# ctb/khmer

Measured on NVIDIA B200. Metric: kmers_per_sec_countgraph_k20_N4, higher is better.
Workload: dtype u8

## Files before the change

khmer_b200/csrc/kmgpu_api.cu:

```cuda
#include <algorithm>
#include <cstdarg>
#include <cstdio>
#include <cstdlib>
#include <cstring>
#include <chrono>
#include <functional>
#include <mutex>
#include <string>
#include <unordered_map>
#include <vector>

#include "../../include/kmgpu.h"
#include "kmgpu_kernels.cuh"
#include "kmgpu_group.cuh"

using namespace kmgpu;

static thread_local std::string g_err;

static int fail(int code, const char* fmt, ...)
{
    char buf[1024];
    va_list ap;
    va_start(ap, fmt);
// ... 942 lines not shown
        for (const Part& pt : parts) {
            const Input& in = pt.in;
            if (in.n_pos == 0) continue;
            const unsigned gt = n_tiles(in.n_pos);
            if (src == 1) k_bigscan2<TWOBIT, 1><<<gt, THREADS, 0, st>>>(h->dev, H, in, sg, h->d_htkeys.p, slots - 1, n_cross ? 1 : 0, h->d_events.p,
                                                                       (unsigned long long)cap, h->d_ctrl, pt.pos_off, MM, PP, pred ? 1 : 0);
            else if (H.kind == TWOBIT) k_bigscan2<TWOBIT, 0><<<gt, THREADS, 0, st>>>(h->dev, H, in, sg, h->d_htkeys.p, slots - 1, n_cross ? 1 : 0, h->d_events.p,
                                                                                   (unsigned long long)cap, h->d_ctrl, pt.pos_off, MM, PP, pred ? 1 : 0);
            else k_bigscan2<MURMUR, 0><<<gt, THREADS, 0, st>>>(h->dev, H, in, sg, h->d_htkeys.p, slots - 1, n_cross ? 1 : 0, h->d_events.p,
                                                             (unsigned long long)cap, h->d_ctrl, pt.pos_off, MM, PP, pred ? 1 : 0);
            h->all_launches += 1;
        }
    }
    SatBits sb;
    memset(&sb, 0, sizeof sb);
    for (int i = 0; i < h->nt && i < F_MAXT; i++) sb.t[i] = h->d_satbits[i].p;
    for (size_t pi = 0; pi < parts.size(); pi++) {
        const Part& pt = parts[pi];
        Input in = pt.in;
        if (in.n_pos == 0 || rehash) continue;
        if (pi + 1 < parts.size()) in.n_pos = std::min<uint32_t>(in.n_pos, parts[pi + 1].pos_off - pt.pos_off);
        const uint32_t* bins = h->d_bins.p + pt.pos_off;
        unsigned gb = (in.n_pos + 255) / 256;
        if (src == 1) k_bigscan<TWOBIT, 1><<<gb, 256, 0, st>>>(h->nt, H, in, bins, stride, sb, h->d_htkeys.p, slots - 1, n_cross ? 1 : 0,
                                                                h->d_events.p, (unsigned long long)cap, h->d_ctrl, pt.pos_off);
        else if (H.kind == TWOBIT) k_bigscan<TWOBIT, 0><<<gb, 256, 0, st>>>(h->nt, H, in, bins, stride, sb, h->d_htkeys.p, slots - 1,
                                                                            n_cross ? 1 : 0, h->d_events.p, (unsigned long long)cap, h->d_ctrl, pt.pos_off);
        else k_bigscan<MURMUR, 0><<<gb, 256, 0, st>>>(h->nt, H, in, bins, stride, sb, h->d_htkeys.p, slots - 1, n_cross ? 1 : 0,
                                                      h->d_events.p, (unsigned long long)cap, h->d_ctrl, pt.pos_off);
        h->all_launches += 1;
    }
    CK(cudaGetLastError());
    CKR(read_ctrl(h));
    const uint64_t n_rec = h->h_ctrl->n_events;
    lap("scan done (n_rec)", n_rec);
    if (n_rec > cap) return fail(KMGPU_ECUDA, "internal: bigcount scan overflow");
    if (n_rec == 0) return KMGPU_OK;
    const unsigned gr = (unsigned)((n_rec + 255) / 256);
    uint32_t* Tarr = nullptr;
    if (n_cross) {
        CKR(h->d_sel.ensure(std::max<uint64_t>(3 * slots, WS_MIN)));
        CKR(h->d_recslot.ensure(std::max<uint64_t>(n_rec * h->nt, 4 * WS_MIN)));
        SelState ss{h->d_sel.p, h->d_sel.p + slots, h->d_sel.p + 2 * slots};
        const unsigned gsl = (unsigned)((slots + 255) / 256);
        k_sel_slots<<<gr, 256, 0, st>>>(h->d_events.p, n_rec, h->dev, h->d_htkeys.p, slots - 1, h->d_recslot.p);
        k_sel_init<<<gsl, 256, 0, st>>>(h->d_htkeys.p, h->d_htvals.p, slots, ss);
        int top = 0;
        while (top < 31 && (1ull << (top + 1)) <= (uint64_t)n_pos) top++;
        for (int bit = top; bit >= 0; bit--) {
            k_sel_count<<<gr, 256, 0, st>>>(h->d_events.p, n_rec, h->nt, h->d_recslot.p, bit, ss);
            k_sel_update<<<gsl, 256, 0, st>>>(slots, bit, ss);
        }
        h->all_launches += 2 + 2 * (top + 1);
        Tarr = ss.prefix;
    }
    uint64_t evslots = pow2_at_least(2 * n_rec);
    CKR(h->d_evkeys.ensure(std::max<uint64_t>(evslots, WS_MIN)));
    CKR(h->d_evvals.ensure(std::max<uint64_t>(2 * evslots, 2 * WS_MIN)));
    CK(cudaMemsetAsync(h->d_evkeys.p, 0xFF, evslots * 8, st));
    CK(cudaMemsetAsync(h->d_evvals.p, 0, evslots * 4, st));
    CK(cudaMemsetAsync(h->d_evvals.p + evslots, 0xFF, evslots * 4, st));
    CK(cudaMemsetAsync(&h->d_ctrl->n_unique, 0, sizeof(unsigned long long), st));
    CK(cudaMemsetAsync(&h->d_ctrl->n_events, 0, sizeof(unsigned long long), st));
    EvTable ev{h->d_evkeys.p, h->d_evvals.p, h->d_evvals.p + evslots, evslots - 1};
    k_ev_decide<<<gr, 256, 0, st>>>(h->d_events.p, n_rec, h->nt, h->d_recslot.p, Tarr, n_cross ? 1 : 0, ev, h->d_ctrl);
    h->all_launches += 1;
    CK(cudaGetLastError());
    CKR(read_ctrl(h));
    const uint64_t n_distinct = h->h_ctrl->n_unique;
    lap("decided (n_distinct)", n_distinct);
    if (n_distinct == 0) return KMGPU_OK;
    CKR(h->d_evout.ensure(std::max<uint64_t>(n_distinct, WS_MIN / 4)));
    CKR(h->h_evout.ensure(std::max<uint64_t>(n_distinct, WS_MIN / 4)));
    k_ev_compact<<<(unsigned)((evslots + 255) / 256), 256, 0, st>>>(ev, h->d_evout.p, h->d_ctrl);
    h->all_launches += 1;
    CK(cudaGetLastError());
    CK(cudaMemcpyAsync(h->h_evout.p, h->d_evout.p, n_distinct * sizeof(EvOut), cudaMemcpyDeviceToHost, st));
    CK(cudaStreamSynchronize(st));
    std::vector<EvOut> evs(h->h_evout.p, h->h_evout.p + n_distinct);
    std::sort(evs.begin(), evs.end(), [](const EvOut& a, const EvOut& b) { return a.first < b.first; });
    for (const EvOut& e : evs) big_events(h, e.hash, e.count);
    return KMGPU_OK;
}

static bool plan_buckets(const kmgpu_sketch* h, uint32_t n_pos, BucketLayout* L)
{
    if (!env_u64("KMGPU_BUCKETS", 1)) return false;
    memset(L, 0, sizeof *L);
    L->n_tables = h->nt;
    uint64_t cap = 0, total = 0;
    for (int i = 0; i < h->nt; i++) {
        if (h->sizes[i] > 0xFFFFFFFEull - 128) return false;
        uint64_t nb = (h->sizes[i] + BKT_BINS - 1) / BKT_BINS;
        if (nb > (uint64_t)BKT_MAX_BUCKETS) return false;
        L->first[i] = (uint32_t)total;
        total += nb;
        uint64_t expect = nb == 1 ? n_pos : (uint64_t)((double)n_pos * BKT_BINS / (double)h->sizes[i]) + 1;
        cap = std::max(cap, expect + expect / 4 + 2048);
    }
    L->first[h->nt] = (uint32_t)total;
    cap = std::min<uint64_t>(cap, (uint64_t)n_pos);
    if (uint64_t forced = env_u64("KMGPU_BUCKET_CAP", 0)) cap = forced;
    if (cap > 65535 || cap == 0) return false;
    L->cap = (uint32_t)cap;
    return true;
}

template <int KIND>
static void launch_apply(unsigned g, cudaStream_t st, const SketchDev& S, const BucketLayout& L, const unsigned long long* rec, const uint32_t* cur,
                         uint32_t* newbits, uint64_t* binlist, unsigned long long list_cap, Ctrl* ctrl, int want_cross, const SatBits& sb)
{
    k_apply<KIND><<<g, 1024, BKT_APPLY_SMEM, st>>>(S, L, rec, cur, newbits, binlist, list_cap, ctrl, want_cross, sb);
}

typedef std::function<int()> Between;

#include "kmgpu_group_host.inc"

static int ingest_chunk_delta(kmgpu_sketch* h, const std::vector<DeltaPass>& passes, int src, HashCfg H, const std::vector<Part>& parts, const Pred& P,
                              bool pred, const SketchDev* M, ChunkResult* res, const Between& between)
{
    cudaStream_t st = h->stream;
    uint32_t n_pos = 0;
    for (const Part& pt : parts) n_pos = std::max(n_pos, pt.pos_off + pt.in.n_pos);
    const uint64_t stride = ((uint64_t)n_pos + 7) & ~7ull;
    CKR(h->d_bins.ensure((size_t)h->nt * stride));
    uint64_t total_bins = 0, max_span = 0;
    for (int i = 0; i < h->nt; i++) total_bins += h->sizes[i];
    for (const DeltaPass& p : passes) max_span = std::max<uint64_t>(max_span, p.hi - p.lo);
    const uint64_t list_cap = std::max<uint64_t>(1, std::min<uint64_t>((uint64_t)h->nt * n_pos, total_bins));
    CKR(h->d_binlist.ensure(list_cap));
    size_t need_lanes = h->kind == BIT ? ((max_span + 127) / 128) * 8 + 8 : ((max_span + 7) & ~7ull) + 8;
    if (h->d_delta.cap < need_lanes) h->delta_zeroed = 0;
    CKR(h->d_delta.ensure(need_lanes));
    if (h->delta_zeroed < h->d_delta.cap) {
        CK(cudaMemsetAsync(h->d_delta.p, 0, h->d_delta.cap * 2, st));
        h->delta_zeroed = h->d_delta.cap;
    }
    CK(cudaMemsetAsync(h->d_ctrl, 0, sizeof(Ctrl), st));
    CK(cudaEventRecord(h->ev0, st));
    const int want_cross = h->kind == BYTE && h->use_bigcount;
    if (want_cross && !h->satbits_valid) {
        for (int i = 0; i < h->nt; i++) {
            uint64_t groups = (h->sizes[i] + 7) / 8;
            CKR(h->d_satbits[i].ensure(groups));
            k_build_satbits<<<(unsigned)std::min<uint64_t>((groups + 255) / 256, 148 * 16), 256, 0, st>>>(h->dev.tables[i], groups, h->d_satbits[i].p);
            h->all_launches += 1;
        }
        h->satbits_valid = true;
    }
    bool kmers_counted = false;
    BucketLayout BL;
    bool use_buckets = plan_buckets(h, n_pos, &BL);
    if (use_buckets) {
        if (!h->bucket_attr_set) {
            CK(cudaFuncSetAttribute(k_bucketize<BKT_TILE, BKT_PER>, cudaFuncAttributeMaxDynamicSharedMemorySize, (int)bkt_sort_smem(BKT_TILE)));
            CK(cudaFuncSetAttribute(k_apply<BYTE>, cudaFuncAttributeMaxDynamicSharedMemorySize, (int)BKT_APPLY_SMEM));
            CK(cudaFuncSetAttribute(k_apply<NIBBLE>, cudaFuncAttributeMaxDynamicSharedMemorySize, (int)BKT_APPLY_SMEM));
            CK(cudaFuncSetAttribute(k_apply<BIT>, cudaFuncAttributeMaxDynamicSharedMemorySize, (int)BKT_APPLY_SMEM));
            h->bucket_attr_set = true;
        }
        const uint32_t n_buckets = BL.first[h->nt];
        if (h->d_records.ensure((size_t)n_buckets * BL.cap) != KMGPU_OK) {
            cudaGetLastError();
            use_buckets = false;
        }
    }
    if (use_buckets) {
        const uint32_t n_buckets = BL.first[h->nt];
        CKR(h->d_cursors.ensure(n_buckets));
        const size_t nb_words = (n_pos + 31) / 32;
        CKR(h->d_newbits.ensure(nb_words));
        CK(cudaMemsetAsync(h->d_cursors.p, 0, (size_t)n_buckets * 4, st));
        CK(cudaMemsetAsync(h->d_newbits.p, 0, nb_words * 4, st));
    }
    for (const Part& pt : parts) {
        const Input& in = pt.in;
        if (pt.ready) CK(cudaStreamWaitEvent(st, pt.ready, 0));
        if (in.n_pos == 0) continue;
        uint32_t* bins = h->d_bins.p + pt.pos_off;
        const unsigned g = n_tiles(in.n_pos);
        const SketchDev& MS = M ? *M : h->dev;
        if (src == 1) launch_hashbins<TWOBIT, 1>(pred, g, st, h->dev, MS, H, P, in, bins, stride, h->d_ctrl);
        else if (H.kind == TWOBIT) launch_hashbins<TWOBIT, 0>(pred, g, st, h->dev, MS, H, P, in, bins, stride, h->d_ctrl);
        else launch_hashbins<MURMUR, 0>(pred, g, st, h->dev, MS, H, P, in, bins, stride, h->d_ctrl);
        if (use_buckets)
            k_bucketize<BKT_TILE, BKT_PER><<<dim3((in.n_pos + BKT_TILE - 1) / BKT_TILE, h->nt), BKT_TILE / BKT_PER, bkt_sort_smem(BKT_TILE), st>>>(
                bins, stride, in.n_pos, pt.pos_off, BL, h->d_records.p, h->d_cursors.p, h->d_ctrl);
        h->ingest_launches += use_buckets ? 2 : 1;
        h->all_launches += use_buckets ? 2 : 1;
    }
    if (use_buckets) {
        const uint32_t n_buckets = BL.first[h->nt];
        const size_t nb_words = (n_pos + 31) / 32;
        SatBits sb;
        memset(&sb, 0, sizeof sb);
        if (want_cross)
            for (int i = 0; i < h->nt; i++) sb.t[i] = h->d_satbits[i].p;
        if (h->kind == BYTE) launch_apply<BYTE>(n_buckets, st, h->dev, BL, h->d_records.p, h->d_cursors.p, h->d_newbits.p, h->d_binlist.p, list_cap, h->d_ctrl, want_cross, sb);
        else if (h->kind == NIBBLE) launch_apply<NIBBLE>(n_buckets, st, h->dev, BL, h->d_records.p, h->d_cursors.p, h->d_newbits.p, h->d_binlist.p, list_cap, h->d_ctrl, 0, sb);
        else launch_apply<BIT>(n_buckets, st, h->dev, BL, h->d_records.p, h->d_cursors.p, h->d_newbits.p, h->d_binlist.p, list_cap, h->d_ctrl, 0, sb);
        k_popc<<<(unsigned)std::min<size_t>((nb_words + 255) / 256, 148 * 8), 256, 0, st>>>(h->d_newbits.p, nb_words, &h->d_ctrl->n_unique);
        CK(cudaEventRecord(h->ev1, st));
        CK(cudaGetLastError());
        if (between) CKR(between());
        CKR(read_ctrl(h));
        float ms = 0;
        CK(cudaEventElapsedTime(&ms, h->ev0, h->ev1));
        h->ingest_ms += ms;
        h->ingest_launches += 2;
        h->all_launches += 2;
        Ctrl c = *h->h_ctrl;
        res->n_kmers += c.n_kmers;
        kmers_counted = true;
        if (!c.overflow) {
            if (c.n_events > list_cap) return fail(KMGPU_ECUDA, "internal: bin list overflow");
            h->n_occupied += c.n_z0;
            if (c.n_zbits) {
                h->n_unique += c.n_unique;
                res->n_new += c.n_unique;
                res->have_newbits = true;
            }
            if (want_cross && c.n_sat) CKR(resolve_bigcount_delta(h, src, H, parts, n_pos, stride, c.n_events, c.n_cross));
            return KMGPU_OK;
        }
        if (env_u64("KMGPU_DEBUG", 0)) fprintf(stderr, "[kmgpu] bucket overflow (cap %u, %u positions): chunk redone by the delta passes\n", BL.cap, n_pos);
        CK(cudaMemsetAsync(h->d_ctrl, 0, sizeof(Ctrl), st));
        CK(cudaEventRecord(h->ev0, st));
    }
    const Between none;
    const Between& between2 = kmers_counted ? none : between;
    const unsigned gs = (n_pos + 2047) / 2048;
    for (const DeltaPass& p : passes) {
        const int pass_id = passes.size() <= 64 ? (int)(&p - passes.data()) : -1;
        if (h->kind == BIT) {
            k_scatter<true><<<gs, 256, 0, st>>>(h->d_bins.p + (size_t)p.table * stride, n_pos, p.lo, p.hi, h->d_delta.p);
            unsigned gb = (unsigned)(((uint64_t)(p.hi - p.lo) + 128 * 256 - 1) / (128 * 256));
            k_fold_bits<<<gb, 256, 0, st>>>(h->dev.tables[p.table], p.table, p.lo, p.hi, h->d_delta.p, h->d_binlist.p, list_cap, h->d_ctrl, pass_id);
            continue;
        }
        k_scatter<false><<<gs, 256, 0, st>>>(h->d_bins.p + (size_t)p.table * stride, n_pos, p.lo, p.hi, h->d_delta.p);
        unsigned gf = (unsigned)(((uint64_t)(p.hi - p.lo) + 2047) / 2048);
        if (h->kind == BYTE)
            k_fold<BYTE><<<gf, 256, 0, st>>>(h->dev.tables[p.table], p.table, p.lo, p.hi, h->d_delta.p, h->d_binlist.p, list_cap, h->d_ctrl, want_cross,
                                             want_cross ? h->d_satbits[p.table].p : nullptr, pass_id);
        else
            k_fold<NIBBLE><<<gf, 256, 0, st>>>(h->dev.tables[p.table], p.table, p.lo, p.hi, h->d_delta.p, h->d_binlist.p, list_cap, h->d_ctrl, 0, nullptr, pass_id);
    }
    CK(cudaEventRecord(h->ev1, st));
    CK(cudaGetLastError());
    if (between2) CKR(between2());
    CKR(read_ctrl(h));
    float ms = 0;
    CK(cudaEventElapsedTime(&ms, h->ev0, h->ev1));
    h->ingest_ms += ms;
    h->ingest_launches += 2 * passes.size();
    h->all_launches += 2 * passes.size();
    Ctrl c = *h->h_ctrl;
    if (c.n_events > list_cap) return fail(KMGPU_ECUDA, "internal: bin list overflow");
    if (!kmers_counted) res->n_kmers += c.n_kmers;
    h->n_occupied += c.n_z0;
    const uint64_t n_list = c.n_events;
    if (c.n_zbits) {
        size_t nb_words = (n_pos + 31) / 32;
        CKR(h->d_newbits.ensure(nb_words));
        CK(cudaMemsetAsync(h->d_newbits.p, 0, nb_words * 4, st));
        CK(cudaMemsetAsync(&h->d_ctrl->n_unique, 0, sizeof(unsigned long long), st));
        const uint64_t cold_min = env_u64("KMGPU_COLD_MIN_NEW", 8ull << 20);
        if (passes.size() <= 64 && c.n_zbits >= cold_min) {
            unsigned long long* sl = reinterpret_cast<unsigned long long*>(h->d_htkeys.p);
            uint64_t seg0 = 0;
            for (size_t pi = 0; pi < passes.size(); pi++) {
                uint64_t seg1 = seg0 + c.pass_list_end[pi];
                if (seg1 > seg0) {
                    const DeltaPass& p = passes[pi];
                    const uint32_t span = p.hi - p.lo;
                    if (span <= (1u << 26) && env_u64("KMGPU_COLD_RANK", 1)) {
                        const uint32_t n_words = (span + 31) / 32;
                        const unsigned gw = (n_words + 1023) / 1024;
                        const uint64_t n_ent = seg1 - seg0;
                        CKR(h->d_rank.ensure((size_t)n_words * 2 + gw));
                        CKR(h->d_htkeys.ensure((n_ent + 1) / 2));
                        uint2* rec = reinterpret_cast<uint2*>(h->d_rank.p);
                        uint32_t* sums = h->d_rank.p + (size_t)n_words * 2;
                        uint32_t* minpos = reinterpret_cast<uint32_t*>(h->d_htkeys.p);
                        CK(cudaMemsetAsync(rec, 0, (size_t)n_words * 8, st));
                        CK(cudaMemsetAsync(minpos, 0xFF, n_ent * 4, st));
                        unsigned gl = (unsigned)std::min<uint64_t>((n_ent + 255) / 256, 148 * 8);
                        k_rank_setbits<<<gl, 256, 0, st>>>(h->d_binlist.p + seg0, n_ent, p.lo, rec);
                        k_rank_sums<<<gw, 256, 0, st>>>(rec, n_words, sums);
                        k_rank_scan<<<1, 1024, 0, st>>>(sums, gw);
                        k_rank_prefix<<<gw, 256, 0, st>>>(rec, n_words, sums);
                        k_rank_replay<<<(n_pos + 2047) / 2048, 256, 0, st>>>(h->d_bins.p + (size_t)p.table * stride, n_pos, p.lo, p.hi, rec, minpos);
                        k_rank_mark<<<gl, 256, 0, st>>>(minpos, n_ent, h->d_newbits.p, h->d_ctrl);
                        h->all_launches += 6;
                        seg0 = seg1;
                        continue;
                    }
                    uint64_t slots = pow2_at_least(2 * (seg1 - seg0));
                    CKR(h->d_htkeys.ensure(slots));
                    sl = reinterpret_cast<unsigned long long*>(h->d_htkeys.p);
                    CK(cudaMemsetAsync(sl, 0xFF, slots * 8, st));
                    unsigned gl = (unsigned)std::min<uint64_t>((seg1 - seg0 + 255) / 256, 148 * 8);
                    k_pk_register<<<gl, 256, 0, st>>>(h->d_binlist.p + seg0, seg1 - seg0, p.table, sl, slots - 1, nullptr);
                    k_pk_replay<<<(n_pos + 1023) / 1024, 256, 0, st>>>(h->d_bins.p + (size_t)p.table * stride, n_pos, p.lo, p.hi, sl,
                                                                    slots - 1, nullptr);
                    unsigned gm = (unsigned)std::min<uint64_t>((slots + 255) / 256, 148 * 8);
                    k_pk_mark<<<gm, 256, 0, st>>>(sl, slots, h->d_newbits.p, h->d_ctrl);
                    h->all_launches += 3;
                }
                seg0 = seg1;
            }
        } else {
        PkLayout L;
        memset(&L, 0, sizeof L);
        uint64_t total_slots = 0;
        for (int i = 0; i < h->nt; i++) {
            if (!c.n_new_t[i]) continue;
            uint64_t sl = pow2_at_least(2 * c.n_new_t[i]);
            L.base[i] = total_slots;
            L.mask[i] = sl - 1;
            total_slots += sl;
        }
        L.use_filter = c.n_zbits < (uint64_t)h->nt * FILTER_BITS / 4;
        {
            uint64_t mx = 0;
            for (int i = 0; i < h->nt; i++) mx = std::max<uint64_t>(mx, c.n_new_t[i]);
            uint64_t fb = 1u << 15;
            while (fb < 32 * mx && fb < FILTER_BITS) fb <<= 1;
            L.filter_bits = (uint32_t)fb;
        }
        CKR(h->d_htkeys.ensure(total_slots));
        CK(cudaMemsetAsync(h->d_htkeys.p, 0xFF, total_slots * 8, st));
        if (L.use_filter) {
            CKR(h->d_filter.ensure((size_t)h->nt * FILTER_WORDS));
            CK(cudaMemsetAsync(h->d_filter.p, 0, (size_t)h->nt * (L.filter_bits >> 5) * 4, st));
        }
        unsigned long long* sl = reinterpret_cast<unsigned long long*>(h->d_htkeys.p);
        unsigned gl = (unsigned)std::min<uint64_t>((n_list + 255) / 256, 148 * 8);
        k_pk_register_all<<<gl, 256, 0, st>>>(h->d_binlist.p, n_list, L, sl, h->d_filter.p);
// ... 2128 lines not shown
```

khmer_b200/csrc/kmgpu_kernels.cuh:

```cuda
#pragma once
#include "kmgpu_device.cuh"

namespace kmgpu {

struct Ctrl {
    unsigned long long n_kmers;
    unsigned long long n_z0;
    unsigned long long n_zbits;
    unsigned long long n_allsat;
    unsigned long long n_sat;
    unsigned long long n_cross;
    unsigned long long n_unique;
    unsigned long long n_events;
    unsigned long long non_acgt;
    unsigned long long n_new_t[32];
    unsigned long long pass_list_end[64];
    unsigned long long overflow;
    unsigned long long queue_overflow;
};

constexpr uint32_t F_CONSUMED = 1u << 31;
constexpr int F_MAXT = 10;
constexpr uint64_t FILTER_BITS = 1ull << 23;
constexpr uint64_t FILTER_WORDS = FILTER_BITS / 32;
// ... 1062 lines not shown
    __shared__ unsigned s_w[32];
    __shared__ unsigned s_carry;
    if (threadIdx.x == 0) s_carry = 0;
    __syncthreads();
    for (uint32_t base = 0; base < n; base += 1024) {
        uint32_t i = base + threadIdx.x;
        unsigned v = i < n ? sums[i] : 0, incl = v;
        const unsigned lane = threadIdx.x & 31, wid = threadIdx.x >> 5;
#pragma unroll
        for (int o = 1; o < 32; o <<= 1) {
            unsigned t = __shfl_up_sync(0xffffffffu, incl, o);
            if (lane >= (unsigned)o) incl += t;
        }
        if (lane == 31) s_w[wid] = incl;
        __syncthreads();
        unsigned before = s_carry;
        for (unsigned w = 0; w < wid; w++) before += s_w[w];
        if (i < n) sums[i] = before + incl - v;
        __syncthreads();
        if (threadIdx.x == 1023) s_carry = before + incl;
        __syncthreads();
    }
}

__global__ void __launch_bounds__(256) k_rank_prefix(uint2* rec, uint32_t n_words, const uint32_t* __restrict__ sums)
{
    const uint32_t w0 = (blockIdx.x * 256u + threadIdx.x) * 4u;
    unsigned c[4], tot = 0;
#pragma unroll
    for (int j = 0; j < 4; j++) {
        c[j] = w0 + j < n_words ? __popc(rec[w0 + j].x) : 0;
        tot += c[j];
    }
    unsigned incl = tot;
    const unsigned lane = threadIdx.x & 31, wid = threadIdx.x >> 5;
#pragma unroll
    for (int o = 1; o < 32; o <<= 1) {
        unsigned t = __shfl_up_sync(0xffffffffu, incl, o);
        if (lane >= (unsigned)o) incl += t;
    }
    __shared__ unsigned s[8];
    if (lane == 31) s[wid] = incl;
    __syncthreads();
    unsigned at = sums[blockIdx.x] + incl - tot;
    for (unsigned w = 0; w < wid; w++) at += s[w];
#pragma unroll
    for (int j = 0; j < 4; j++) {
        if (w0 + j < n_words) rec[w0 + j].y = at;
        at += c[j];
    }
}

__global__ void __launch_bounds__(256)
k_rank_replay(const uint32_t* __restrict__ bins, uint32_t n_pos, uint32_t lo, uint32_t hi, const uint2* __restrict__ rec, uint32_t* minpos)
{
    const uint32_t p0 = (blockIdx.x * 256u + threadIdx.x) * 8u;
    if (p0 >= n_pos) return;
    uint32_t v[8];
    if (p0 + 8 <= n_pos) {
        uint4 a = __ldcs(reinterpret_cast<const uint4*>(bins + p0));
        uint4 b = __ldcs(reinterpret_cast<const uint4*>(bins + p0 + 4));
        v[0] = a.x; v[1] = a.y; v[2] = a.z; v[3] = a.w; v[4] = b.x; v[5] = b.y; v[6] = b.z; v[7] = b.w;
    } else {
#pragma unroll
        for (int j = 0; j < 8; j++) v[j] = p0 + j < n_pos ? __ldcs(bins + p0 + j) : BIN_NONE;
    }
    const uint32_t span = hi - lo;
    uint2 r[8];
#pragma unroll
    for (int j = 0; j < 8; j++) {
        v[j] -= lo;
        r[j] = v[j] < span ? __ldcg(&rec[v[j] >> 5]) : make_uint2(0, 0);
    }
#pragma unroll
    for (int j = 0; j < 8; j++) {
        const uint32_t bit = 1u << (v[j] & 31);
        if (r[j].x & bit) atomicMin(&minpos[r[j].y + __popc(r[j].x & (bit - 1))], p0 + j);
    }
}

__global__ void k_rank_mark(const uint32_t* __restrict__ minpos, uint64_t n, uint32_t* newbits, Ctrl* ctrl)
{
    unsigned cnt = 0;
    for (uint64_t i = blockIdx.x * (uint64_t)blockDim.x + threadIdx.x; i < n; i += (uint64_t)gridDim.x * blockDim.x) {
        uint32_t p = minpos[i];
        if (p == 0xFFFFFFFFu) continue;
        uint32_t bit = 1u << (p & 31);
        uint32_t old = atomicOr(&newbits[p >> 5], bit);
        cnt += !(old & bit);
    }
    cnt = __reduce_add_sync(0xffffffffu, cnt);
    if ((threadIdx.x & 31) == 0 && cnt) atomicAdd(&ctrl->n_unique, (unsigned long long)cnt);
}

struct PkLayout {
    uint64_t base[F_MAXT];
    uint64_t mask[F_MAXT];
    int use_filter;
    uint32_t filter_bits;
};

__global__ void k_pk_register_all(const uint64_t* __restrict__ binlist, uint64_t n, PkLayout L, unsigned long long* slots, uint32_t* filter)
{
    for (uint64_t i = blockIdx.x * (uint64_t)blockDim.x + threadIdx.x; i < n; i += (uint64_t)gridDim.x * blockDim.x) {
        uint64_t e = binlist[i];
        if (!(e & BL_NEW)) continue;
        int t = (int)(e & 255u);
        uint32_t bin = (uint32_t)((e & 0xFFFFFFFFFFFFull) >> 8);
        unsigned long long fresh = ((unsigned long long)bin << 32) | 0xFFFFFFFFull;
        unsigned long long* tb = slots + L.base[t];
        uint64_t s = pk_slot0(bin, L.mask[t]);
        while (true) {
            unsigned long long prev = atomicCAS(&tb[s], PK_EMPTY, fresh);
            if (prev == PK_EMPTY || (uint32_t)(prev >> 32) == bin) break;
            s = (s + 1) & L.mask[t];
        }
        if (L.use_filter) atomicOr(&filter[t * (L.filter_bits >> 5) + ((bin & (L.filter_bits - 1)) >> 5)], 1u << (bin & 31));
    }
}

__global__ void __launch_bounds__(256)
k_pk_replay_all(const uint32_t* __restrict__ bins, uint64_t stride, int n_tables, uint32_t n_pos, PkLayout L, unsigned long long* slots,
                const uint32_t* __restrict__ filter)
{
    uint32_t p = blockIdx.x * 256u + threadIdx.x;
    if (p >= n_pos) return;
    uint32_t b[F_MAXT];
    bool act[F_MAXT];
#pragma unroll
    for (int t = 0; t < F_MAXT; t++) b[t] = t < n_tables ? __ldcs(&bins[t * stride + p]) : BIN_NONE;
    if (b[0] == BIN_NONE) return;
    const uint32_t fmask = L.filter_bits - 1, fwords = L.filter_bits >> 5;
#pragma unroll
    for (int t = 0; t < F_MAXT; t++) {
        act[t] = t < n_tables && L.mask[t] != 0;
        if (act[t] && L.use_filter) act[t] = (__ldg(&filter[t * fwords + ((b[t] & fmask) >> 5)]) >> (b[t] & 31)) & 1u;
    }
#pragma unroll
    for (int t = 0; t < F_MAXT; t++) {
        if (!act[t]) continue;
        unsigned long long* tb = slots + L.base[t];
        uint64_t s = pk_slot0(b[t], L.mask[t]);
        pk_finish(tb, L.mask[t], s, __ldcg(&tb[s]), b[t], p);
    }
}

struct SatBits {
    const uint8_t* t[F_MAXT];
};

constexpr int BKT_SHIFT = 15;
constexpr uint32_t BKT_BINS = 1u << BKT_SHIFT;
constexpr int BKT_MAX_BUCKETS = 6144;
constexpr int BKT_PER = 16;
constexpr int BKT_TILE = 16384;
constexpr size_t BKT_APPLY_SMEM = (size_t)BKT_BINS * 2 + (size_t)BKT_BINS * 4;
constexpr size_t bkt_sort_smem(int tile) { return (size_t)tile * 8 + (size_t)BKT_MAX_BUCKETS * 12; }

struct BucketLayout {
    uint32_t first[F_MAXT + 1];
    uint32_t cap;
    int n_tables;
};

template <int T, int PER>
__global__ void __launch_bounds__(T / PER, 1)
k_bucketize(const uint32_t* __restrict__ bins, uint64_t stride, uint32_t n_pos, uint32_t pos_base, BucketLayout L,
            unsigned long long* __restrict__ records, uint32_t* __restrict__ cursors, Ctrl* ctrl)
{
    constexpr int NT = T / PER;
    constexpr int BPT = (BKT_MAX_BUCKETS + NT - 1) / NT;
    extern __shared__ __align__(16) unsigned char bk_raw[];
    uint2* stage = reinterpret_cast<uint2*>(bk_raw);
    uint2* run = stage + T;
    uint32_t* hist = reinterpret_cast<uint32_t*>(run + BKT_MAX_BUCKETS);
    __shared__ uint32_t s_warp[32];
    __shared__ uint32_t s_total;
    const int t = blockIdx.y;
    const uint32_t nb = L.first[t + 1] - L.first[t];
    const uint32_t p0 = blockIdx.x * (uint32_t)T;
    const uint32_t tid = threadIdx.x;
    uint32_t bin[PER], rk[PER / 2];
    const uint32_t* src = bins + (size_t)t * stride;
#pragma unroll
    for (int j = 0; j < PER; j++) {
        uint32_t p = p0 + j * NT + tid;
        bin[j] = p < n_pos ? __ldcs(src + p) : BIN_NONE;
    }
    for (uint32_t i = tid; i < nb; i += NT) hist[i] = 0;
    __syncthreads();
#pragma unroll
    for (int j = 0; j < PER; j++) {
        uint32_t r = bin[j] != BIN_NONE ? atomicAdd(&hist[bin[j] >> BKT_SHIFT], 1u) : 0u;
        if (j & 1) rk[j >> 1] |= r << 16; else rk[j >> 1] = r;
    }
    __syncthreads();
    uint32_t c[BPT], mine = 0;
#pragma unroll
    for (int q = 0; q < BPT; q++) {
        uint32_t b = tid * BPT + q;
        c[q] = b < nb ? hist[b] : 0;
        mine += c[q];
    }
    uint32_t incl = mine;
    const uint32_t lane = tid & 31, wid = tid >> 5;
#pragma unroll
    for (int o = 1; o < 32; o <<= 1) {
        uint32_t v = __shfl_up_sync(0xffffffffu, incl, o);
        if (lane >= (uint32_t)o) incl += v;
    }
    if (lane == 31) s_warp[wid] = incl;
    __syncthreads();
    if (wid == 0) {
        uint32_t v = lane < NT / 32 ? s_warp[lane] : 0, w = v;
#pragma unroll
        for (int o = 1; o < 32; o <<= 1) {
            uint32_t u = __shfl_up_sync(0xffffffffu, w, o);
            if (lane >= (uint32_t)o) w += u;
        }
        s_warp[lane] = w - v;
        if (lane == 31) s_total = w;
    }
    __syncthreads();
    uint32_t at = s_warp[wid] + incl - mine, gbase[BPT];
#pragma unroll
    for (int q = 0; q < BPT; q++) {
        uint32_t b = tid * BPT + q;
        if (b < nb) run[b].x = at;
        gbase[q] = c[q] ? atomicAdd(&cursors[L.first[t] + b], c[q]) : 0u;
        at += c[q];
    }
    __syncthreads();
#pragma unroll
    for (int j = 0; j < PER; j++) {
        if (bin[j] == BIN_NONE) continue;
        const uint32_t b = bin[j] >> BKT_SHIFT;
        const uint32_t r = (j & 1) ? rk[j >> 1] >> 16 : rk[j >> 1] & 0xFFFFu;
        stage[run[b].x + r] = make_uint2(((uint32_t)(j * NT + tid) << BKT_SHIFT) | (bin[j] & (BKT_BINS - 1)), (b << 16) | r);
    }
#pragma unroll
    for (int q = 0; q < BPT; q++) {
        uint32_t b = tid * BPT + q;
        if (b < nb) run[b].y = gbase[q];
    }
    __syncthreads();
    const uint32_t total = s_total;
    const size_t base = (size_t)L.first[t] * L.cap;
    bool over = false;
    for (uint32_t s = tid; s < total; s += NT) {
        const uint2 m = stage[s];
        const uint32_t b = m.y >> 16, idx = run[b].y + (m.y & 0xFFFFu);
        if (idx < L.cap)
            records[base + (size_t)b * L.cap + idx] = ((unsigned long long)(pos_base + p0 + (m.x >> BKT_SHIFT)) << BKT_SHIFT) | (m.x & (BKT_BINS - 1));
        else
            over = true;
    }
    if (over) atomicExch(&ctrl->overflow, 1ull);
}

__global__ void k_popc(const uint32_t* __restrict__ words, uint64_t n, unsigned long long* out)
{
    unsigned cnt = 0;
    for (uint64_t i = blockIdx.x * (uint64_t)blockDim.x + threadIdx.x; i < n; i += (uint64_t)gridDim.x * blockDim.x) cnt += __popc(words[i]);
    cnt = __reduce_add_sync(0xffffffffu, cnt);
    if ((threadIdx.x & 31) == 0 && cnt) atomicAdd(out, (unsigned long long)cnt);
}

template <int KIND>
__global__ void __launch_bounds__(1024, 1)
k_apply(SketchDev S, BucketLayout L, const unsigned long long* __restrict__ records, const uint32_t* __restrict__ cursors,
        uint32_t* __restrict__ newbits, uint64_t* __restrict__ binlist, unsigned long long list_cap, Ctrl* ctrl, int want_cross, SatBits sb)
{
    extern __shared__ __align__(16) uint32_t ap_smem[];
    uint32_t* cnt = ap_smem;
    uint32_t* minpos = ap_smem + BKT_BINS / 2;
    if (ctrl->overflow) return;
    const uint32_t n = cursors[blockIdx.x];
    if (n == 0) return;
    int t = 0;
    uint32_t first_t = 0;
    const uint8_t* sat = nullptr;
#pragma unroll
    for (int i = 0; i < F_MAXT; i++)
        if (i < L.n_tables && blockIdx.x >= L.first[i]) {
            t = i;
            first_t = L.first[i];
            sat = sb.t[i];
        }
    const uint32_t bin0 = (blockIdx.x - first_t) << BKT_SHIFT;
    const uint32_t tid = threadIdx.x;
    const uint64_t size = S.sizes[t];
    uint8_t* table = S.tables[t];
    constexpr int GPT = BKT_BINS / 8 / 1024;
    uint64_t oldv[GPT];
#pragma unroll
    for (int q = 0; q < GPT; q++) {
        const uint32_t b0 = bin0 + (q * 1024 + tid) * 8;
        oldv[q] = 0;
        if (b0 < size) {
            if (KIND == BYTE) oldv[q] = __ldcs(reinterpret_cast<const unsigned long long*>(table + b0));
            else if (KIND == NIBBLE) oldv[q] = __ldcs(reinterpret_cast<const uint32_t*>(table + (b0 >> 1)));
            else oldv[q] = __ldcs(table + (b0 >> 3));
        }
    }
    {
        uint4* z = reinterpret_cast<uint4*>(cnt);
        for (uint32_t i = tid; i < BKT_BINS / 8; i += 1024) z[i] = make_uint4(0, 0, 0, 0);
        uint4* f = reinterpret_cast<uint4*>(minpos);
        for (uint32_t i = tid; i < BKT_BINS / 4; i += 1024) f[i] = make_uint4(~0u, ~0u, ~0u, ~0u);
    }
    __syncthreads();
    const unsigned long long* src = records + (size_t)blockIdx.x * L.cap;
    constexpr int RIF = 16;
    for (uint32_t e0 = 0; e0 < n; e0 += RIF * 1024) {
        unsigned long long v[RIF];
#pragma unroll
        for (int j = 0; j < RIF; j++) {
            uint32_t e = e0 + j * 1024 + tid;
            v[j] = e < n ? __ldcs(src + e) : ~0ull;
        }
#pragma unroll
        for (int j = 0; j < RIF; j++) {
            if (v[j] == ~0ull) continue;
            uint32_t lb = (uint32_t)v[j] & (BKT_BINS - 1);
            atomicAdd(&cnt[lb >> 1], (lb & 1) ? 0x10000u : 1u);
            atomicMin(&minpos[lb], (uint32_t)(v[j] >> BKT_SHIFT));
        }
    }
    __syncthreads();
    unsigned n_new = 0, n_sat = 0, n_cross = 0;
#pragma unroll
    for (int q = 0; q < GPT; q++) {
        const uint32_t g = q * 1024 + tid;
        const uint32_t b0 = bin0 + g * 8;
        if (b0 >= size) continue;
        const uint4 c4 = reinterpret_cast<const uint4*>(cnt)[g];
        if (!(c4.x | c4.y | c4.z | c4.w)) continue;
        const uint32_t cw[4] = {c4.x, c4.y, c4.z, c4.w};
        unsigned newm = 0, crossm = 0;
        if (KIND == BYTE) {
            const uint64_t old64 = oldv[q];
            uint64_t new64 = old64;
            unsigned fullm = 0;
#pragma unroll
            for (int j = 0; j < 8; j++) {
                uint32_t m = (cw[j >> 1] >> ((j & 1) * 16)) & 0xFFFFu;
                if (!m) continue;
                uint32_t s = (uint32_t)(old64 >> (8 * j)) & 255u, tt = s + m, nv = tt > 255u ? 255u : tt;
                new64 = (new64 & ~(255ull << (8 * j))) | ((uint64_t)nv << (8 * j));
                newm |= (unsigned)(s == 0) << j;
                n_sat += tt > 255u;
                crossm |= (unsigned)(tt >= 255u && s < 255u) << j;
                fullm |= (unsigned)(nv == 255u) << j;
            }
            *reinterpret_cast<uint64_t*>(table + b0) = new64;
            if (want_cross && fullm) {
                unsigned m = 0;
#pragma unroll
                for (int j = 0; j < 8; j++) m |= (unsigned)(((new64 >> (8 * j)) & 255u) == 255u) << j;
                const_cast<uint8_t*>(sat)[b0 >> 3] = (uint8_t)m;
            }
            n_cross += __popc(crossm);
            if (want_cross && crossm) {
#pragma unroll
                for (int j = 0; j < 8; j++) {
                    if (!((crossm >> j) & 1u)) continue;
                    unsigned long long at = atomicAdd(&ctrl->n_events, 1ull);
                    if (at < list_cap) binlist[at] = BL_CROSS | (((old64 >> (8 * j)) & 255ull) << 48) | ht_key((uint64_t)(b0 + j), t);
                }
            }
        } else if (KIND == NIBBLE) {
            const uint32_t old32 = (uint32_t)oldv[q];
            uint32_t new32 = old32;
#pragma unroll
            for (int j = 0; j < 8; j++) {
                uint32_t m = (cw[j >> 1] >> ((j & 1) * 16)) & 0xFFFFu;
                if (!m) continue;
                const uint32_t sh = (j >> 1) * 8 + ((j & 1) ? 0 : 4);
                uint32_t s = (old32 >> sh) & 15u, tt = s + m, nv = tt > 15u ? 15u : tt;
                new32 = (new32 & ~(15u << sh)) | (nv << sh);
                newm |= (unsigned)(s == 0) << j;
            }
            *reinterpret_cast<uint32_t*>(table + (b0 >> 1)) = new32;
        } else {
            const unsigned old8 = (unsigned)oldv[q];
            unsigned touched = 0;
#pragma unroll
            for (int j = 0; j < 8; j++) touched |= (unsigned)(((cw[j >> 1] >> ((j & 1) * 16)) & 0xFFFFu) != 0) << j;
            newm = touched & ~old8;
            if (newm) table[b0 >> 3] = (uint8_t)(old8 | touched);
        }
        n_new += __popc(newm);
#pragma unroll
        for (int j = 0; j < 8; j++) {
            if (!((newm >> j) & 1u)) continue;
            const uint32_t p = minpos[g * 8 + j];
            atomicOr(&newbits[p >> 5], 1u << (p & 31));
        }
    }
    __shared__ unsigned s_tot[3];
    if (tid < 3) s_tot[tid] = 0;
    __syncthreads();
    n_new = __reduce_add_sync(0xffffffffu, n_new);
    n_sat = __reduce_add_sync(0xffffffffu, n_sat);
    n_cross = __reduce_add_sync(0xffffffffu, n_cross);
    if ((tid & 31) == 0) {
// ... 270 lines not shown
```

Before: 21.82 billion.

## Shrink bucketize shared-memory staging and double tile size to 32K positions

Reworks the bucketize kernel's shared-memory layout. The staging buffer now holds 4-byte entries plus a 2-byte bucket id instead of 8-byte pairs, and the per-bucket arrays are sized to the actual bucket count. This frees enough shared memory for a 32768-position tile with a fixed 1024 threads. Bins are re-read from global memory (L2) in the scatter phase instead of being held in registers, which cuts register pressure at the cost of a second read. Larger tiles mean fewer blocks and fewer global cursor atomics per position, and a 16K-tile fallback covers cases where the bucket count exceeds the shared-memory limit.

```diff
diff --git a/khmer_b200/csrc/kmgpu_api.cu b/khmer_b200/csrc/kmgpu_api.cu
--- a/khmer_b200/csrc/kmgpu_api.cu
+++ b/khmer_b200/csrc/kmgpu_api.cu
@@ -1118,9 +1118,14 @@
     bool kmers_counted = false;
     BucketLayout BL;
     bool use_buckets = plan_buckets(h, n_pos, &BL);
+    uint32_t nb_max = 0;
+    if (use_buckets)
+        for (int i = 0; i < h->nt; i++) nb_max = std::max(nb_max, BL.first[i + 1] - BL.first[i]);
+    const bool big_tile = bkt_sort_smem(BKT_TILE_BIG, nb_max) <= BKT_SMEM_LIMIT;
     if (use_buckets) {
         if (!h->bucket_attr_set) {
-            CK(cudaFuncSetAttribute(k_bucketize<BKT_TILE, BKT_PER>, cudaFuncAttributeMaxDynamicSharedMemorySize, (int)bkt_sort_smem(BKT_TILE)));
+            CK(cudaFuncSetAttribute(k_bucketize<BKT_TILE_BIG>, cudaFuncAttributeMaxDynamicSharedMemorySize, (int)BKT_SMEM_LIMIT));
+            CK(cudaFuncSetAttribute(k_bucketize<BKT_TILE>, cudaFuncAttributeMaxDynamicSharedMemorySize, (int)bkt_sort_smem(BKT_TILE, BKT_MAX_BUCKETS)));
             CK(cudaFuncSetAttribute(k_apply<BYTE>, cudaFuncAttributeMaxDynamicSharedMemorySize, (int)BKT_APPLY_SMEM));
             CK(cudaFuncSetAttribute(k_apply<NIBBLE>, cudaFuncAttributeMaxDynamicSharedMemorySize, (int)BKT_APPLY_SMEM));
             CK(cudaFuncSetAttribute(k_apply<BIT>, cudaFuncAttributeMaxDynamicSharedMemorySize, (int)BKT_APPLY_SMEM));
@@ -1150,8 +1155,11 @@
         if (src == 1) launch_hashbins<TWOBIT, 1>(pred, g, st, h->dev, MS, H, P, in, bins, stride, h->d_ctrl);
         else if (H.kind == TWOBIT) launch_hashbins<TWOBIT, 0>(pred, g, st, h->dev, MS, H, P, in, bins, stride, h->d_ctrl);
         else launch_hashbins<MURMUR, 0>(pred, g, st, h->dev, MS, H, P, in, bins, stride, h->d_ctrl);
-        if (use_buckets)
-            k_bucketize<BKT_TILE, BKT_PER><<<dim3((in.n_pos + BKT_TILE - 1) / BKT_TILE, h->nt), BKT_TILE / BKT_PER, bkt_sort_smem(BKT_TILE), st>>>(
+        if (use_buckets && big_tile)
+            k_bucketize<BKT_TILE_BIG><<<dim3((in.n_pos + BKT_TILE_BIG - 1) / BKT_TILE_BIG, h->nt), BKT_THREADS, bkt_sort_smem(BKT_TILE_BIG, nb_max), st>>>(
+                bins, stride, in.n_pos, pt.pos_off, BL, h->d_records.p, h->d_cursors.p, h->d_ctrl);
+        else if (use_buckets)
+            k_bucketize<BKT_TILE><<<dim3((in.n_pos + BKT_TILE - 1) / BKT_TILE, h->nt), BKT_THREADS, bkt_sort_smem(BKT_TILE, nb_max), st>>>(
                 bins, stride, in.n_pos, pt.pos_off, BL, h->d_records.p, h->d_cursors.p, h->d_ctrl);
         h->ingest_launches += use_buckets ? 2 : 1;
         h->all_launches += use_buckets ? 2 : 1;
diff --git a/khmer_b200/csrc/kmgpu_kernels.cuh b/khmer_b200/csrc/kmgpu_kernels.cuh
--- a/khmer_b200/csrc/kmgpu_kernels.cuh
+++ b/khmer_b200/csrc/kmgpu_kernels.cuh
@@ -1238,10 +1238,11 @@
 constexpr int BKT_SHIFT = 15;
 constexpr uint32_t BKT_BINS = 1u << BKT_SHIFT;
 constexpr int BKT_MAX_BUCKETS = 6144;
-constexpr int BKT_PER = 16;
-constexpr int BKT_TILE = 16384;
+constexpr int BKT_THREADS = 1024;
 constexpr size_t BKT_APPLY_SMEM = (size_t)BKT_BINS * 2 + (size_t)BKT_BINS * 4;
-constexpr size_t bkt_sort_smem(int tile) { return (size_t)tile * 8 + (size_t)BKT_MAX_BUCKETS * 12; }
+constexpr size_t bkt_sort_smem(int tile, uint32_t nb) { return (size_t)tile * 6 + (size_t)nb * 8; }
+constexpr int BKT_TILE_BIG = 32768, BKT_TILE = 16384;
+constexpr size_t BKT_SMEM_LIMIT = 227 * 1024 - 1024;
 
 struct BucketLayout {
     uint32_t first[F_MAXT + 1];
@@ -1249,43 +1250,52 @@
     int n_tables;
 };
 
-template <int T, int PER>
-__global__ void __launch_bounds__(T / PER, 1)
+template <int T>
+__global__ void __launch_bounds__(BKT_THREADS, 1)
 k_bucketize(const uint32_t* __restrict__ bins, uint64_t stride, uint32_t n_pos, uint32_t pos_base, BucketLayout L,
             unsigned long long* __restrict__ records, uint32_t* __restrict__ cursors, Ctrl* ctrl)
 {
-    constexpr int NT = T / PER;
+    constexpr int NT = BKT_THREADS, PER = T / NT;
     constexpr int BPT = (BKT_MAX_BUCKETS + NT - 1) / NT;
+    static_assert(T <= 32768, "ranks and positions in the tile are kept in 16 / 15 bits");
+    const int t = blockIdx.y;
+    const uint32_t nb = L.first[t + 1] - L.first[t];
     extern __shared__ __align__(16) unsigned char bk_raw[];
-    uint2* stage = reinterpret_cast<uint2*>(bk_raw);
-    uint2* run = stage + T;
-    uint32_t* hist = reinterpret_cast<uint32_t*>(run + BKT_MAX_BUCKETS);
+    uint32_t* stage = reinterpret_cast<uint32_t*>(bk_raw);
+    uint32_t* runoff = stage + T;
+    uint32_t* gbase = runoff + nb;
+    uint16_t* sbkt = reinterpret_cast<uint16_t*>(gbase + nb);
     __shared__ uint32_t s_warp[32];
     __shared__ uint32_t s_total;
-    const int t = blockIdx.y;
-    const uint32_t nb = L.first[t + 1] - L.first[t];
     const uint32_t p0 = blockIdx.x * (uint32_t)T;
     const uint32_t tid = threadIdx.x;
-    uint32_t bin[PER], rk[PER / 2];
-    const uint32_t* src = bins + (size_t)t * stride;
-#pragma unroll
-    for (int j = 0; j < PER; j++) {
-        uint32_t p = p0 + j * NT + tid;
-        bin[j] = p < n_pos ? __ldcs(src + p) : BIN_NONE;
-    }
-    for (uint32_t i = tid; i < nb; i += NT) hist[i] = 0;
-    __syncthreads();
-#pragma unroll
-    for (int j = 0; j < PER; j++) {
-        uint32_t r = bin[j] != BIN_NONE ? atomicAdd(&hist[bin[j] >> BKT_SHIFT], 1u) : 0u;
-        if (j & 1) rk[j >> 1] |= r << 16; else rk[j >> 1] = r;
+    const uint32_t* src = bins + (size_t)t * stride + p0;
+    const uint32_t n_tile = min(n_pos - p0, (uint32_t)T);
+    uint32_t rk[PER / 2];
+    for (uint32_t i = tid; i < nb; i += NT) runoff[i] = 0;
+    __syncthreads();
+    constexpr int G = PER < 8 ? PER : 8;
+#pragma unroll
+    for (int j0 = 0; j0 < PER; j0 += G) {
+        uint32_t bin[G];
+#pragma unroll
+        for (int j = 0; j < G; j++) {
+            uint32_t p = (j0 + j) * NT + tid;
+            bin[j] = p < n_tile ? __ldcg(src + p) : BIN_NONE;
+        }
+#pragma unroll
+        for (int j = 0; j < G; j++) {
+            uint32_t r = bin[j] != BIN_NONE ? atomicAdd(&runoff[bin[j] >> BKT_SHIFT], 1u) : 0u;
+            if (j & 1) rk[(j0 + j) >> 1] |= r << 16; else rk[(j0 + j) >> 1] = r;
+        }
+        asm volatile("" ::: "memory");
     }
     __syncthreads();
     uint32_t c[BPT], mine = 0;
 #pragma unroll
     for (int q = 0; q < BPT; q++) {
         uint32_t b = tid * BPT + q;
-        c[q] = b < nb ? hist[b] : 0;
+        c[q] = b < nb ? runoff[b] : 0;
         mine += c[q];
     }
     uint32_t incl = mine;
@@ -1308,36 +1318,41 @@
         if (lane == 31) s_total = w;
     }
     __syncthreads();
-    uint32_t at = s_warp[wid] + incl - mine, gbase[BPT];
+    uint32_t at = s_warp[wid] + incl - mine;
 #pragma unroll
     for (int q = 0; q < BPT; q++) {
         uint32_t b = tid * BPT + q;
-        if (b < nb) run[b].x = at;
-        gbase[q] = c[q] ? atomicAdd(&cursors[L.first[t] + b], c[q]) : 0u;
+        if (b < nb) runoff[b] = at;
+        if (c[q]) gbase[b] = atomicAdd(&cursors[L.first[t] + b], c[q]);
         at += c[q];
     }
     __syncthreads();
 #pragma unroll
-    for (int j = 0; j < PER; j++) {
-        if (bin[j] == BIN_NONE) continue;
-        const uint32_t b = bin[j] >> BKT_SHIFT;
-        const uint32_t r = (j & 1) ? rk[j >> 1] >> 16 : rk[j >> 1] & 0xFFFFu;
-        stage[run[b].x + r] = make_uint2(((uint32_t)(j * NT + tid) << BKT_SHIFT) | (bin[j] & (BKT_BINS - 1)), (b << 16) | r);
-    }
-#pragma unroll
-    for (int q = 0; q < BPT; q++) {
-        uint32_t b = tid * BPT + q;
-        if (b < nb) run[b].y = gbase[q];
+    for (int j0 = 0; j0 < PER; j0 += G) {
+        uint32_t bin[G];
+#pragma unroll
+        for (int j = 0; j < G; j++) {
+            const uint32_t p = (j0 + j) * NT + tid;
+            bin[j] = p < n_tile ? __ldcg(src + p) : BIN_NONE;
+        }
+#pragma unroll
+        for (int j = 0; j < G; j++) {
+            if (bin[j] == BIN_NONE) continue;
+            const uint32_t b = bin[j] >> BKT_SHIFT, q = (j0 + j) >> 1;
+            const uint32_t s = runoff[b] + ((j & 1) ? rk[q] >> 16 : rk[q] & 0xFFFFu);
+            stage[s] = (((j0 + j) * NT + tid) << BKT_SHIFT) | (bin[j] & (BKT_BINS - 1));
+            sbkt[s] = (uint16_t)b;
+        }
+        asm volatile("" ::: "memory");
     }
     __syncthreads();
     const uint32_t total = s_total;
-    const size_t base = (size_t)L.first[t] * L.cap;
+    unsigned long long* dst = records + (size_t)L.first[t] * L.cap;
     bool over = false;
     for (uint32_t s = tid; s < total; s += NT) {
-        const uint2 m = stage[s];
-        const uint32_t b = m.y >> 16, idx = run[b].y + (m.y & 0xFFFFu);
+        const uint32_t m = stage[s], b = sbkt[s], idx = gbase[b] + (s - runoff[b]);
         if (idx < L.cap)
-            records[base + (size_t)b * L.cap + idx] = ((unsigned long long)(pos_base + p0 + (m.x >> BKT_SHIFT)) << BKT_SHIFT) | (m.x & (BKT_BINS - 1));
+            dst[(size_t)b * L.cap + idx] = ((unsigned long long)(pos_base + p0 + (m >> BKT_SHIFT)) << BKT_SHIFT) | (m & (BKT_BINS - 1));
         else
             over = true;
     }
```

Measured after the change: 21.46 billion, median of 6. -1.6%, worse.
